# jayHuggie/PathTracer_CUDA_Interactive

Hardware: AMD Instinct MI355X
Metric: Msamples/sec (rays x spp x bounces = intersect() calls per second), scenes/cbox/cbox.xml 640x480 spp=64 (higher is better)
Workload: dtype f32

## Files before the change

pathtracer_cuda_interactive_amd/csrc/pt_kernels.h:

```cpp
#pragma once

#include <hip/hip_runtime.h>

#include <type_traits>

#include "pt_layout.h"
#include "pt_leaf_sweep.h"
#include "pt_math.h"
#include "pt_path_bank.h"
#include "pt_sweep_layout.h"
#include "pt_temporal.h"
#include "pt_trace.h"

namespace ptk {

using namespace ptl;


#ifndef PT_BLOCK
#define PT_BLOCK 256
#endif
constexpr int kBlock = PT_BLOCK;
constexpr uint32_t kMaxChunk = 256;

__device__ __forceinline__ uint32_t lane_rank(unsigned long long mask) {
    return __builtin_amdgcn_mbcnt_hi((uint32_t)(mask >> 32), __builtin_amdgcn_mbcnt_lo((uint32_t)mask, 0u));
}

__device__ __forceinline__ unsigned long long wave_sum(unsigned long long v) {
    for (int off = 32; off > 0; off >>= 1) v += __shfl_down(v, off, 64);
    return v;
}


constexpr int kCounterStride = 32;

struct WorkFeed {
    uint32_t cur, end;
    uint32_t region;
    uint32_t tried;
    bool exhausted;
};

__device__ __forceinline__ uint32_t region_rows(const RenderDev& rp, uint32_t region) {
    const uint32_t first = region * (uint32_t)rp.rows_per_region;
    const uint32_t nrows = (uint32_t)rp.num_rows;
    return first >= nrows ? 0u : min((uint32_t)rp.rows_per_region, nrows - first);
}

__device__ __forceinline__ void feed_init(WorkFeed& f, const RenderDev& rp) {
    f.cur = 0; f.end = 0; f.tried = 0; f.exhausted = false;
    const uint32_t xcc = (uint32_t)__builtin_amdgcn_s_getreg(6164) & 15u;
    f.region = xcc % (uint32_t)rp.num_regions;
}

__device__ __forceinline__ void feed_reserve(WorkFeed& f, const RenderDev& rp, uint32_t* work_counters, int lane) {
    while (f.cur >= f.end && !f.exhausted) {
        const uint32_t total = region_rows(rp, f.region) * (uint32_t)rp.width * (uint32_t)rp.spp_pass;
        const uint32_t chunk = rp.chunk;
        uint32_t base = 0;
        if (lane == 0) base = atomicAdd(&work_counters[f.region * kCounterStride], chunk);
        base = __builtin_amdgcn_readfirstlane(base);
        if (base < total) {
            f.cur = base;
            f.end = min(base + chunk, total);
        } else if (++f.tried >= (uint32_t)rp.num_regions) {
            f.exhausted = true;
        } else {
            f.region = (f.region + 1) % (uint32_t)rp.num_regions;
        }
    }
}

struct PathStart {
    ptd::Ray ray;
    ptm::Pcg rng;
    uint32_t sample_index;
};

struct PathIndex {
    int col, j;
    int32_t img_width;
    uint64_t stream;
    uint32_t sample_index;
};

template <bool LIST = false>
__device__ __forceinline__ PathIndex path_index(const RenderDev& rp, uint32_t region, uint32_t item) {
    const uint32_t npix_r = region_rows(rp, region) * (uint32_t)rp.width;
    uint32_t s_local, rr;
    int i;
    if (rp.row_major) {
        const uint32_t row_s = fastdiv(item, rp.div_width);
        i = (int)(item - row_s * (uint32_t)rp.width);
        rr = fastdiv(row_s, rp.div_spp);
        s_local = row_s - rr * (uint32_t)rp.spp_pass;
    } else {
        s_local = fastdiv(item, (int)region == rp.short_region ? rp.div_npix_last : rp.div_npix_full);
        const uint32_t pix_r = item - s_local * npix_r;
        rr = fastdiv(pix_r, rp.div_width);
        i = (int)(pix_r - rr * (uint32_t)rp.width);
    }
    const uint32_t local_row = region * (uint32_t)rp.rows_per_region + rr;
    uint32_t img_row = local_row;
    int col = i;
    if (LIST) {
        const uint32_t e = rp.list[local_row];
        img_row = fastdiv(e, rp.div_img_width);
        col = (int)(e - img_row * (uint32_t)rp.img_width);
    }
    const int32_t img_width = LIST ? rp.img_width : rp.width;
    const int j = rp.row_begin + (int)img_row * rp.row_step;
    const uint64_t pixel_index = (uint64_t)j * (uint64_t)img_width + (uint64_t)col;
    PathIndex px;
    px.col = col;
    px.j = j;
    px.img_width = img_width;
    px.stream = pixel_index * (uint64_t)rp.stream_stride + (uint64_t)(rp.sample_base + (int)s_local);
    px.sample_index = s_local * rp.npix + local_row * (uint32_t)rp.width + (uint32_t)i;
    return px;
}

template <bool LIST = false>
__device__ __forceinline__ PathStart start_path(const RenderDev& rp, uint32_t region, uint32_t item) {
    const PathIndex px = path_index<LIST>(rp, region, item);
    PathStart ps;
    ps.rng = ptm::pcg_init(px.stream, rp.seed);
    const float ru = ptm::pcg_float(ps.rng);
    const float u = ((float)px.col + ru) / (float)px.img_width;
    const float rv = ptm::pcg_float(ps.rng);
    const float v = ((float)px.j + rv) / (float)rp.height;
    ps.ray = ptd::primary_ray(rp, u, v);
    ps.sample_index = px.sample_index;
    return ps;
}

struct TraceKernelArgs {
    SceneDev scn; RenderDev rp; LdsPlan lp; float4* samples; uint32_t* work_counter; unsigned long long* counters;
};
template <bool WORDS>
__device__ __forceinline__ RenderDev reload_render_args() {
    typedef const __attribute__((address_space(4))) unsigned char* KernargPtr;
    KernargPtr p = (KernargPtr)__builtin_amdgcn_kernarg_segment_ptr();
    asm volatile("" : "+s"(p));
    if (WORDS) {
        struct Words { uint32_t w[sizeof(RenderDev) / 4]; };
        typedef const __attribute__((address_space(4))) uint32_t* WordPtr;
        WordPtr q = (WordPtr)(p + offsetof(TraceKernelArgs, rp));
        Words v;
#pragma unroll
        for (uint32_t i = 0; i < sizeof(RenderDev) / 4; i++) v.w[i] = q[i];
        return __builtin_bit_cast(RenderDev, v);
    }
    RenderDev r;
    __builtin_memcpy(&r, (const void*)(p + offsetof(TraceKernelArgs, rp)), sizeof(RenderDev));
    return r;
}

#ifndef PT_PATH_BANK
#define PT_PATH_BANK 1
#endif
constexpr bool path_bank_on(int res, int spec, bool nee, bool list, int thresh, int inner) {
    return PT_PATH_BANK && (res == 1 || res == 2) && spec == 2 && !nee && !list && thresh == 40 && inner == 162;
}

__device__ __forceinline__ void stage_to_lds(void* dst, const void* src, uint32_t bytes) {
    float4* d = reinterpret_cast<float4*>(dst);
    const float4* s = reinterpret_cast<const float4*>(src);
    for (uint32_t i = threadIdx.x; i < bytes / 16; i += blockDim.x) d[i] = s[i];
}

#ifndef PT_LDS_NODE_STRIDE
#define PT_LDS_NODE_STRIDE 64
#endif
constexpr uint32_t kLdsNodeStride = PT_LDS_NODE_STRIDE;
__device__ __forceinline__ void stage_nodes_to_lds(void* dst, const DNode* src, uint32_t n) {
    const float4* s = reinterpret_cast<const float4*>(src);
    for (uint32_t i = threadIdx.x; i < n * 4; i += blockDim.x)
        *reinterpret_cast<float4*>(reinterpret_cast<unsigned char*>(dst) + (i >> 2) * kLdsNodeStride + (i & 3) * 16) = s[i];
}

template <int RES>
__device__ __forceinline__ ptd::SceneView make_scene_view(const SceneDev& scn, const LdsPlan& lp, unsigned char* smem) {
    ptd::SceneView sv;
    sv.top_nodes = nullptr;
    sv.top_count = 0;
    if (RES == 1 || RES == 2) {
        const uint32_t oct_pitch = oct_table_pitch((uint32_t)scn.num_nodes, kLdsNodeStride);
        if (RES == 2) {
            for (uint32_t o = 0; o < 8; o++)
                stage_nodes_to_lds(smem + lp.nodes_off + o * oct_pitch, scn.nodes_oct + (size_t)o * scn.num_nodes, (uint32_t)scn.num_nodes);
        } else {
            stage_nodes_to_lds(smem + lp.nodes_off, scn.nodes, (uint32_t)scn.num_nodes);
        }
        stage_to_lds(smem + lp.prims_off, scn.prims, (uint32_t)scn.num_prims * sizeof(DPrim));
        stage_to_lds(smem + lp.normals_off, scn.normals, (uint32_t)scn.num_prims * sizeof(DNormals));
        stage_to_lds(smem + lp.mats_off, scn.materials, (uint32_t)scn.num_materials * sizeof(DMaterial));
        stage_to_lds(smem + lp.emis_off, scn.emission, (uint32_t)scn.num_emission * sizeof(DEmission));
        __syncthreads();
        sv.nodes = reinterpret_cast<const DNode*>(smem + lp.nodes_off);
        sv.prims = reinterpret_cast<const DPrim*>(smem + lp.prims_off);
        sv.normals = reinterpret_cast<const DNormals*>(smem + lp.normals_off);
        sv.materials = reinterpret_cast<const DMaterial*>(smem + lp.mats_off);
        sv.emission = reinterpret_cast<const DEmission*>(smem + lp.emis_off);
        sv.node_stride = kLdsNodeStride;
        sv.oct_stride = RES == 2 ? oct_pitch : 0u;
    } else {
        if (RES == 3) {
            stage_to_lds(smem + lp.nodes_off, scn.nodes, lp.top_count * (uint32_t)sizeof(DNode));
            __syncthreads();
            sv.top_nodes = reinterpret_cast<const DNode*>(smem + lp.nodes_off);
            sv.top_count = lp.top_count;
        }
        sv.nodes = scn.nodes; sv.prims = scn.prims; sv.normals = scn.normals;
        sv.materials = scn.materials; sv.emission = scn.emission;
        sv.node_stride = sizeof(DNode);
        sv.oct_stride = 0;
    }
    sv.lights = scn.lights;
    sv.num_emission = scn.num_emission;
    sv.root_ref = scn.root_ref;
    sv.fixed_order = scn.fixed_order;
    sv.ref_nodes = scn.ref_nodes; sv.ref_path = scn.ref_path; sv.ref_anc = scn.ref_anc; sv.ref_levels = scn.ref_levels;
    sv.bg = ptm::mk(scn.bg[0], scn.bg[1], scn.bg[2]);
    return sv;
}

constexpr int kCounterSlots = 64;
constexpr int kSlotStride = 16;
constexpr int kTimelineBase = kCounterSlots * kSlotStride;
constexpr int kNumCounters = kTimelineBase + 8 + 2 * 128;

__device__ __forceinline__ unsigned long long* counter_slot(unsigned long long* counters) {
    return counters + (blockIdx.x % kCounterSlots) * kSlotStride;
}

template <bool STATS>
__device__ __forceinline__ void flush_counters(unsigned long long* counters, int lane, uint32_t n_paths, uint32_t n_segs,
                                               const ptd::TravStats& st) {
    const unsigned long long a = wave_sum(n_paths), b = wave_sum(n_segs);
    const unsigned long long c = STATS ? wave_sum(st.nodes) : 0ull, d = STATS ? wave_sum(st.leaves) : 0ull;
    if (lane == 0) {
        unsigned long long* slot = counter_slot(counters);
        atomicAdd(&slot[0], a);
        atomicAdd(&slot[1], b);
        if (STATS) { atomicAdd(&slot[2], c); atomicAdd(&slot[3], d); }
    }
}

template <bool LDS_SCENE, bool PRUNE, bool STATS, bool LIST = false>
__global__ __launch_bounds__(kBlock) void trace_kernel(SceneDev scn, RenderDev rp, LdsPlan lp,
                                                       float4* __restrict__ samples,
                                                       uint32_t* __restrict__ work_counter,
                                                       unsigned long long* __restrict__ counters) {
    extern __shared__ __attribute__((aligned(16))) unsigned char smem[];
    const ptd::SceneView sv = make_scene_view<(LDS_SCENE ? 1 : 0)>(scn, lp, smem);

    const int lane = threadIdx.x & 63;
    const int wave = threadIdx.x >> 6;
    int32_t* stk = reinterpret_cast<int32_t*>(smem + lp.stack_off) + (size_t)wave * scn.stack_cap * 64 + lane;

    WorkFeed feed;
    feed_init(feed, rp);
    bool alive = false;
    ptd::Ray ray;
    ptm::V3 L = ptm::mk(0, 0, 0), T = ptm::mk(1, 1, 1);
    ptm::Pcg rng;
    rng.state = 0; rng.inc = 1;
    int depth = 0;
    uint32_t my_w = 0;
    uint32_t n_paths = 0, n_segs = 0;
    ptd::TravStats st;
    st.nodes = 0; st.leaves = 0;
    ray.org = ptm::mk(0, 0, 0); ray.dir = ptm::mk(0, 0, 1); ray.tnear = 0; ray.tfar = 0;

    for (;;) {
        const unsigned long long need = __ballot(!alive);
        if (need) {
            feed_reserve(feed, rp, work_counter, lane);
            const uint32_t avail = feed.end - feed.cur;
            if (avail) {
                const uint32_t rank = lane_rank(need);
                const uint32_t n = (uint32_t)__popcll(need);
                if (!alive && rank < avail) {
                    const PathStart ps = start_path<LIST>(rp, feed.region, feed.cur + rank);
                    ray = ps.ray;
                    rng = ps.rng;
                    my_w = ps.sample_index;
                    L = ptm::mk(0, 0, 0);
                    T = ptm::mk(1, 1, 1);
                    depth = 0;
                    alive = true;
                    n_paths++;
                }
                feed.cur += min(n, avail);
            }
        }
        if (!__any(alive)) {
            if (feed.exhausted) break;
            continue;
        }
        if (alive) {
            n_segs++;
            const ptd::Hit h = ptd::intersect<PRUNE, STATS>(sv, ray, stk, st);
            bool cont = false;
            if (h.prim < 0) {
                L = L + T * sv.bg;
            } else {
                const ptd::Surface sf = ptd::make_surface<false>(sv, ray, h);
                cont = ptd::shade_and_bounce<false>(sv, sf, ray, rng, L, T, depth, rp.rr_depth);
                depth++;
                if (depth >= rp.max_depth) cont = false;
            }
            if (!cont) {
                samples[my_w] = make_float4(L.x, L.y, L.z, 0.0f);
                alive = false;
            }
// ... 399 lines not shown
```

pathtracer_cuda_interactive_amd/csrc/pt_trace.h:

```cpp
#pragma once

#include <float.h>

#include "pt_layout.h"
#include "pt_math.h"
#include "pt_reg_stack.h"

namespace ptd {

using namespace ptm;
using namespace ptl;

struct Ray {
    V3 org, dir;
    float tnear, tfar;
};

struct Hit {
    float t, u, v;
    int32_t prim;
};

struct TravStats {
    uint32_t nodes, leaves;
// ... 76 lines not shown
    s.reset(t);
    t.redo = false;
    const uint32_t oct = (t.inv.x < 0.0f ? 1u : 0u) | (t.inv.y < 0.0f ? 2u : 0u) | (t.inv.z < 0.0f ? 4u : 0u);
    t.node_off = oct * sv.oct_stride;
}

__device__ __forceinline__ void slab_distances(const float4 a, const float4 b, const float4 c, const V3& o, const V3& inv,
                                               float& ltn, float& ltf, float& rtn, float& rtf) {
    const bool sx = inv.x < 0.0f, sy = inv.y < 0.0f, sz = inv.z < 0.0f;
    float l0x = (a.x - o.x) * inv.x, l1x = (a.w - o.x) * inv.x;
    float l0y = (a.y - o.y) * inv.y, l1y = (b.x - o.y) * inv.y;
    float l0z = (a.z - o.z) * inv.z, l1z = (b.y - o.z) * inv.z;
    ltn = fmax2(fmax2(sx ? l1x : l0x, sy ? l1y : l0y), sz ? l1z : l0z);
    ltf = fmin2(fmin2(sx ? l0x : l1x, sy ? l0y : l1y), sz ? l0z : l1z);
    float r0x = (b.z - o.x) * inv.x, r1x = (c.y - o.x) * inv.x;
    float r0y = (b.w - o.y) * inv.y, r1y = (c.z - o.y) * inv.y;
    float r0z = (c.x - o.z) * inv.z, r1z = (c.w - o.z) * inv.z;
    rtn = fmax2(fmax2(sx ? r1x : r0x, sy ? r1y : r0y), sz ? r1z : r0z);
    rtf = fmin2(fmin2(sx ? r0x : r1x, sy ? r0y : r1y), sz ? r0z : r1z);
}

template <bool PRUNE, bool OCT, class S>
__device__ __forceinline__ void visit_node(const float4 a, const float4 b, const float4 c, const float4 d, const V3& o, Trav& t, const S& s,
                                           const bool fixed_order) {
    const V3 inv = t.inv;
    float ltn, ltf, rtn, rtf;
    if (OCT) {
        ltn = fmax2(fmax2((a.x - o.x) * inv.x, (a.y - o.y) * inv.y), (a.z - o.z) * inv.z);
        ltf = fmin2(fmin2((a.w - o.x) * inv.x, (b.x - o.y) * inv.y), (b.y - o.z) * inv.z);
        rtn = fmax2(fmax2((b.z - o.x) * inv.x, (b.w - o.y) * inv.y), (c.x - o.z) * inv.z);
        rtf = fmin2(fmin2((c.y - o.x) * inv.x, (c.z - o.y) * inv.y), (c.w - o.z) * inv.z);
    } else {
        slab_distances(a, b, c, o, inv, ltn, ltf, rtn, rtf);
    }
    bool hl = ltf >= fmax2(0.0f, ltn);
    bool hr = rtf >= fmax2(0.0f, rtn);
    if (PRUNE) {
        const float lim = t.best.t + t.best.t * 1e-5f;
        hl = hl && !(ltn > lim);
        hr = hr && !(rtn > lim);
    }
    const int32_t L = __builtin_bit_cast(int32_t, d.x);
    const int32_t R = __builtin_bit_cast(int32_t, d.y);
    const bool left_first = S::kLeftFirst || fixed_order || ltn < rtn;
    const bool both = hl && hr;
    const int32_t next = (hl && (!hr || left_first)) ? L : R;
    s.advance(t, both, hl || hr, next, left_first ? R : L);
}

typedef float f4v __attribute__((ext_vector_type(4)));
typedef __attribute__((address_space(3))) const f4v lds_f4v;

template <class P>
__device__ __forceinline__ void ld_node_lds(const P* p, float4& a, float4& b, float4& c, float4& d) {
    const lds_f4v* nd = (const lds_f4v*)p;
    const f4v va = nd[0], vb = nd[1], vc = nd[2], vd = nd[3];
    a = make_float4(va.x, va.y, va.z, va.w); b = make_float4(vb.x, vb.y, vb.z, vb.w);
    c = make_float4(vc.x, vc.y, vc.z, vc.w); d = make_float4(vd.x, vd.y, vd.z, vd.w);
}

template <bool PRUNE, bool OCT, int TOP = 0, class S>
__device__ __forceinline__ void inner_step(const SceneView& sv, const V3& o, Trav& t, const S& s) {
    float4 a, b, c, d;
    if (TOP == 1 && (uint32_t)t.cur < sv.top_count) {
        ld_node_lds(reinterpret_cast<const unsigned char*>(sv.top_nodes) + (uint32_t)t.cur * (uint32_t)sizeof(DNode), a, b, c, d);
    } else {
        const void* nd = reinterpret_cast<const unsigned char*>(sv.nodes) + (OCT ? t.node_off : 0u) + (uint32_t)t.cur * sv.node_stride;
        a = ld4(nd, 0);
        b = ld4(nd, 1);
        c = ld4(nd, 2);
        d = ld4(nd, 3);
    }
    visit_node<PRUNE, OCT>(a, b, c, d, o, t, s, sv.fixed_order != 0);
}

__device__ __forceinline__ bool ref_visits_first(const SceneView& sv, const V3& o, const V3& inv, const int32_t a, const int32_t b) {
    const unsigned long long pa = sv.ref_path[a], pb = sv.ref_path[b];
    const int level = __builtin_ctzll(pa ^ pb);
    const int32_t node = sv.ref_anc[(size_t)a * (size_t)sv.ref_levels + level];
    const DNode* nd = sv.ref_nodes + node;
    float ltn, ltf, rtn, rtf;
    slab_distances(ld4(nd, 0), ld4(nd, 1), ld4(nd, 2), o, inv, ltn, ltf, rtn, rtf);
    const bool left_first = ltn < rtn;
    const bool b_left = ((pb >> level) & 1ull) == 0ull;
    return b_left == left_first;
}

template <bool TRI_ONLY>
__device__ __forceinline__ void leaf_test(const SceneView& sv, const Ray& ray, Trav& t, const int32_t ref, const bool ties) {
    const int32_t prim = ~ref;
    const DPrim* pr = sv.prims + prim;
    const float4 a = ld4(pr, 0);
    const float4 b = ld4(pr, 1);
    const float4 c = ld4(pr, 2);
    const V3 o = ray.org;
    const int32_t info = __builtin_bit_cast(int32_t, c.y);
    if (TRI_ONLY || info >= 0) {
        const V3 p0 = mk(a.x, a.y, a.z), p1 = mk(a.w, b.x, b.y), p2 = mk(b.z, b.w, c.x);
        const V3 e1 = p1 - p0;
        const V3 e2 = p2 - p0;
        const V3 s1 = cross(ray.dir, e2);
        const float divisor = dot(s1, e1);
        if (divisor != 0.0f) {
            const float inv_divisor = rcp_exact(divisor);
            const V3 s = o - p0;
            const float u = dot(s, s1) * inv_divisor;
            const V3 s2 = cross(s, e1);
            const float v = dot(ray.dir, s2) * inv_divisor;
            const float tt = dot(e2, s2) * inv_divisor;
            if (tt > ray.tnear && tt < ray.tfar && u >= 0.0f && v >= 0.0f && u + v <= 1.0f) {
                bool take = tt < t.best.t;
                if (ties && tt == t.best.t && t.best.prim >= 0) {
                    take = ref_visits_first(sv, o, t.inv, t.best.prim, prim);
                }
                if (take) { t.best.t = tt; t.best.u = u; t.best.v = v; t.best.prim = prim; }
            }
        }
    } else {
        const V3 center = mk(a.x, a.y, a.z);
        const float radius = a.w;
        const V3 vv = o - center;
        const float A = dot(ray.dir, ray.dir);
        const float B = 2.0f * dot(ray.dir, vv);
        const float C = dot(vv, vv) - radius * radius;
        float t0 = 0.0f, t1 = 0.0f;
        bool ok = true;
        if (A == 0.0f) {
            if (B == 0.0f) ok = false;
            else { t0 = -C / B; t1 = t0; }
        } else {
            const float disc = B * B - 4.0f * A * C;
            if (disc < 0.0f) ok = false;
            else {
                const float rd = __builtin_sqrtf(disc);
                if (B >= 0.0f) { t0 = (-B - rd) / (2.0f * A); t1 = 2.0f * C / (-B - rd); }
                else { t0 = 2.0f * C / (-B + rd); t1 = (-B + rd) / (2.0f * A); }
            }
        }
        if (ok) {
            if (t0 > t1) { const float tmp = t0; t0 = t1; t1 = tmp; }
            float tt = t0;
            if (t1 >= ray.tnear && t1 < ray.tfar && tt < ray.tnear) tt = t1;
            if (tt >= ray.tnear && tt < ray.tfar) {
                bool take = tt < t.best.t;
                if (ties && tt == t.best.t && t.best.prim >= 0) take = ref_visits_first(sv, o, t.inv, t.best.prim, prim);
                if (take) { t.best.t = tt; t.best.u = 0.0f; t.best.v = 0.0f; t.best.prim = prim; }
            }
        }
    }
}

__device__ __forceinline__ uint32_t leaf_test_slot(const SceneView& sv, const lds_f4v* slots, const Ray& ray, Trav& t, const uint32_t slot) {
    typedef const __attribute__((address_space(3))) unsigned char* LdsBytes;
    static_assert(sizeof(DPrim) == 48, "slot * 48 as two shift-adds (the compiler's own choice is a 64-bit multiply-add)");
    const lds_f4v* pr = (const lds_f4v*)(((LdsBytes)slots + (slot << 5)) + (slot << 4));
    const f4v a = pr[0], b = pr[1], c = pr[2];
    const float link_bits = c.w;
    const uint32_t link = __builtin_bit_cast(uint32_t, link_bits);
    const int32_t prim = (int32_t)(link & 0xffu);
    const V3 o = ray.org;
    const V3 p0 = mk(a.x, a.y, a.z), e1 = mk(a.w, b.x, b.y), e2 = mk(b.z, b.w, c.x);
    const V3 s1 = cross(ray.dir, e2);
    const float divisor = dot(s1, e1);
    if (divisor != 0.0f) {
        const float inv_divisor = rcp_exact(divisor);
        const V3 s = o - p0;
        const float u = dot(s, s1) * inv_divisor;
        const V3 s2 = cross(s, e1);
        const float v = dot(ray.dir, s2) * inv_divisor;
        const float tt = dot(e2, s2) * inv_divisor;
        if (tt > ray.tnear && u >= 0.0f && v >= 0.0f && u + v <= 1.0f) {
            bool take = tt < t.best.t;
            if (tt == t.best.t && t.best.prim >= 0) {
                float dx = ray.dir.x, dy = ray.dir.y, dz = ray.dir.z;
                asm volatile("" : "+v"(dx), "+v"(dy), "+v"(dz));
                const V3 inv = mk(rcp_exact(dx), rcp_exact(dy), rcp_exact(dz));
                take = ref_visits_first(sv, o, inv, t.best.prim, prim);
            }
            if (take) { t.best.t = tt; t.best.u = u; t.best.v = v; t.best.prim = prim; }
        }
    }
    return link >> 8;
}

template <bool TRI_ONLY, bool ANYHIT = false, class S>
__device__ __forceinline__ void leaf_step(const SceneView& sv, const Ray& ray, Trav& t, const S& s, const bool shadow = false,
                                          const bool ties = false) {
    leaf_test<TRI_ONLY>(sv, ray, t, t.cur, ties);
    if (ANYHIT && shadow && t.best.prim >= 0) s.reset(t);
    s.pop(t);
}

template <bool PRUNE, bool STATS>
__device__ __forceinline__ Hit intersect(const SceneView& sv, const Ray& ray, int32_t* stk, TravStats& st) {
    Trav t;
    const LdsStack<int32_t> s{stk};
    stack_init(stk);
    trav_begin(sv, ray, t, s);
    while (t.cur != kDone) {
        while (t.cur >= 0) {
            if (STATS) st.nodes++;
            inner_step<PRUNE, false>(sv, ray.org, t, s);
        }
        if (t.cur != kDone) {
            if (STATS) st.leaves++;
            leaf_step<false>(sv, ray, t, s);
        }
    }
    return t.best;
}

template <bool PRUNE = false>
__device__ __forceinline__ Hit intersect_any_tree(const SceneView& sv, const SceneView& sv_ref, const Ray& ray, int32_t* stk, bool& rerun) {
    Trav t;
    TravStats st;
    st.nodes = 0; st.leaves = 0;
    const LdsStack<int32_t> s{stk};
    stack_init(stk);
    trav_begin(sv, ray, t, s);
    if (!(__builtin_isfinite(t.inv.x) && __builtin_isfinite(t.inv.y) && __builtin_isfinite(t.inv.z))) {
        t.redo = true;
        t.cur = kDone;
    }
    while (t.cur != kDone) {
        while (t.cur >= 0) inner_step<PRUNE, false>(sv, ray.org, t, s);
        if (t.cur != kDone) leaf_step<false>(sv, ray, t, s, false, true);
    }
    rerun = t.redo;
    return t.redo ? intersect<false, false>(sv_ref, ray, stk, st) : t.best;
}

struct Surface {
    V3 p, n;
    int32_t material, light;
};

template <bool TRI_ONLY>
__device__ __forceinline__ Surface make_surface(const SceneView& sv, const Ray& ray, const Hit& h) {
    Surface s;
    const DPrim* pr = sv.prims + h.prim;
    const float4 a = ld4(pr, 0);
    const float4 b = ld4(pr, 1);
    const float4 c = ld4(pr, 2);
    const int32_t info = __builtin_bit_cast(int32_t, c.y);
    s.material = info & 0x7fffffff;
    s.light = __builtin_bit_cast(int32_t, c.z);
    if (TRI_ONLY || info >= 0) {
        const V3 p0 = mk(a.x, a.y, a.z), p1 = mk(a.w, b.x, b.y), p2 = mk(b.z, b.w, c.x);
        const float w = 1.0f - h.u - h.v;
        s.p = p0 * w + p1 * h.u + p2 * h.v;
        const DNormals* nr = sv.normals + h.prim;
        const float4 na = ld4(nr, 0);
        const float4 nb = ld4(nr, 1);
        const float4 nc = ld4(nr, 2);
        const V3 n0 = mk(na.x, na.y, na.z), n1 = mk(na.w, nb.x, nb.y), n2 = mk(nb.z, nb.w, nc.x);
        s.n = normalize(n0 * w + n1 * h.u + n2 * h.v);
    } else {
        const V3 center = mk(a.x, a.y, a.z);
        s.p = ray.org + ray.dir * h.t;
        s.n = normalize(s.p - center);
    }
    return s;
}

__device__ __forceinline__ V3 to_world_about(V3 n, V3 local) {
    V3 fx, fy;
    if (n.z < float(-1 + 1e-6)) {
        fx = mk(0.0f, -1.0f, 0.0f);
        fy = mk(-1.0f, 0.0f, 0.0f);
    } else {
        const float a = rcp_exact(1.0f + n.z);
        const float b = -n.x * n.y * a;
        fx = mk(1.0f - n.x * n.x * a, b, -n.x);
        fy = mk(b, 1.0f - n.y * n.y * a, -n.y);
    }
    return fx * local.x + fy * local.y + n * local.z;
}

__device__ __forceinline__ V3 reflect_about(V3 wi, V3 n) {
    const float k = 2.0f * dot(wi, n);
    return (-wi) + n * k;
}

__device__ __forceinline__ V3 schlick(V3 F0, float cos_theta) {
    const float p5 = pow5(1.0f - cos_theta);
    return F0 + (mk(1.0f, 1.0f, 1.0f) - F0) * p5;
}

__device__ __forceinline__ V3 sample_cos_hemisphere(float ux, float uy) {
    const float phi = kTwoPi * ux;
    const float tmp = sqrt_exact(clamp01(1.0f - uy));
    float sn, cs;
    sincos_det(phi, sn, cs);
    return mk(cs * tmp, sn * tmp, sqrt_exact(clamp01(uy)));
}

__device__ __forceinline__ V3 sample_cos_n_hemisphere(float ux, float uy, float exponent) {
    const float phi = kTwoPi * ux;
    const float cos_theta = pow_det(uy, 1.0f / (exponent + 1.0f));
    const float sin_theta = __builtin_sqrtf(clamp01(1.0f - cos_theta * cos_theta));
    float sn, cs;
    sincos_det(phi, sn, cs);
    return mk(cs * sin_theta, sn * sin_theta, cos_theta);
}

struct LightSample {
    V3 wl;
    float tfar;
// ... 231 lines not shown
```

pathtracer_cuda_interactive_amd/csrc/pt_trace_sweep_body.h:

```cpp
    extern __shared__ __attribute__((aligned(16))) unsigned char smem[];
    constexpr int THRESH = PT_SWEEP_THRESH;
    typedef const __attribute__((address_space(3))) unsigned char* LdsBytes;
    typedef float f2v __attribute__((ext_vector_type(2)));
    typedef const __attribute__((address_space(3))) f2v* LdsF2;
    const uint32_t n_groups = sweep.groups;
    const uint32_t box_pitch = sweep_box_pitch(n_groups);
    const ptd::SceneView sv = make_sweep_view(scn, lp, sweep, smem);
    const ptd::lds_f4v* slots = (const ptd::lds_f4v*)(smem + lp.nodes_off + sweep_slots_off(n_groups));

    const int lane = threadIdx.x & 63;
    const int wave = threadIdx.x >> 6;

    WorkFeed feed;
    feed_init(feed, rp);
    PathBank bank;
    bank_init(bank);
    float bank_dx = 0.0f, bank_dy = 0.0f, bank_dz = 0.0f;
    uint32_t bank_lo = 0, bank_hi = 0;
    bool alive = false;
    ptd::Ray ray;
    ray.org = ptm::mk(0, 0, 0); ray.dir = ptm::mk(0, 0, 1); ray.tnear = 0; ray.tfar = 0;
    ptd::Trav tv;
    tv.inv = ptm::mk(1, 1, 1);
    tv.best.t = 0; tv.best.u = 0; tv.best.v = 0; tv.best.prim = -1;
    tv.cur = 0; tv.stack_state = 0; tv.node_off = 0; tv.redo = false;
    uint32_t hits = 0;
    uint32_t pend = 0;
    ptm::V3 L = ptm::mk(0, 0, 0), T = ptm::mk(1, 1, 1);
    ptm::Pcg rng;
    rng.state = 0; rng.inc = 1;
    int depth = 0;
    uint32_t my_w = 0;
    uint32_t n_paths = 0, n_segs = 0;
    ptd::TravStats st;
    st.nodes = 0; st.leaves = 0;
    ptd::SceneView sv_ref = sv;
    sv_ref.nodes = scn.ref_nodes; sv_ref.root_ref = scn.ref_root_ref; sv_ref.node_stride = sizeof(DNode);
    sv_ref.oct_stride = 0; sv_ref.top_nodes = nullptr; sv_ref.top_count = 0; sv_ref.fixed_order = 0;
    int32_t* redo_stk = scn.redo_stack + ((size_t)(blockIdx.x * (kBlock / 64) + wave) * (size_t)scn.redo_cap) * 64 + lane;

    for (;;) {
        const bool idle = (hits | pend) == 0u;
        const unsigned long long idle_mask = __ballot(idle);
        const bool work_left = bank_work_left(bank, feed.exhausted, feed.cur, feed.end);
        const int n_pend = __popcll(__ballot(idle && (alive || work_left)));
        if (n_pend >= THRESH || idle_mask == ~0ull) {
            if (n_pend == 0) break;
            if (idle && alive && tv.redo) {
                ptd::TravStats st_redo;
                st_redo.nodes = 0; st_redo.leaves = 0;
                ray.tfar = depth == 0 ? __builtin_inff() : FLT_MAX;
                tv.best = ptd::intersect<false, false>(sv_ref, ray, redo_stk, st_redo);
                tv.redo = false;
            }
            if (idle && alive) {
                bool cont = false;
                if (tv.best.prim < 0) {
                    L = L + T * sv.bg;
                } else {
                    const ptd::Surface sf = ptd::make_surface<true>(sv, ray, tv.best);
                    cont = ptd::shade_and_bounce<true, false>(sv, sf, ray, rng, L, T, depth, rp.rr_depth, nullptr);
                    depth++;
                    if (depth >= rp.max_depth) cont = false;
                }
                if (!cont) {
                    samples[my_w] = make_float4(L.x, L.y, L.z, 0.0f);
                    alive = false;
                }
            }
            unsigned long long want = __ballot(idle && !alive);
#pragma nounroll
            for (int round = 0; round < 2 && want; round++) {
                if (bank.left == 0) {
                    feed_reserve(feed, rp, work_counter, lane);
                    if (feed.cur >= feed.end) break;
                    bank_fill(bank, feed.cur, feed.end);
                    const RenderDev rg = reload_render_args<false>();
                    const PathStart ps = start_path<false>(rg, feed.region, bank_item(feed.cur, (uint32_t)lane));
                    bank_dx = ps.ray.dir.x; bank_dy = ps.ray.dir.y; bank_dz = ps.ray.dir.z;
                    bank_lo = (uint32_t)ps.rng.state; bank_hi = (uint32_t)(ps.rng.state >> 32);
                }
                uint32_t first;
                const uint32_t k = bank_take(bank, (uint32_t)__popcll(want), first);
                const uint32_t rank = lane_rank(want);
                const bool take = idle && !alive && rank < k;
                const int src = take ? (int)(first + rank) : lane;
                const float dx = __shfl(bank_dx, src, 64), dy = __shfl(bank_dy, src, 64), dz = __shfl(bank_dz, src, 64);
                const uint32_t lo = __shfl(bank_lo, src, 64), hi = __shfl(bank_hi, src, 64);
                if (take) {
                    const PathIndex px = path_index<false>(rp, feed.region, bank_item(feed.cur, first + rank));
                    ray.org = ptm::mk(rp.cam_origin[0], rp.cam_origin[1], rp.cam_origin[2]);
                    ray.dir = ptm::mk(dx, dy, dz);
                    ray.tnear = 0.0f;
                    rng.state = (uint64_t)hi << 32 | lo;
                    rng.inc = (px.stream << 1u) | 1u;
                    my_w = px.sample_index;
                    L = ptm::mk(0, 0, 0);
                    T = ptm::mk(1, 1, 1);
                    depth = 0;
                    alive = true;
                }
                n_paths += k;
                want = __ballot(idle && !alive);
            }
            n_segs += (uint32_t)__popcll(__ballot(idle && alive));
            if (idle && alive) {
                const ptm::V3 inv = ptm::mk(ptm::rcp_exact(ray.dir.x), ptm::rcp_exact(ray.dir.y), ptm::rcp_exact(ray.dir.z));
                tv.best.t = FLT_MAX; tv.best.u = 0.0f; tv.best.v = 0.0f; tv.best.prim = -1;
                tv.redo = !(__builtin_isfinite(inv.x) && __builtin_isfinite(inv.y) && __builtin_isfinite(inv.z));
                if (!tv.redo) {
                    const uint32_t oct = (inv.x < 0.0f ? 1u : 0u) | (inv.y < 0.0f ? 2u : 0u) | (inv.z < 0.0f ? 4u : 0u);
                    LdsF2 bx = (LdsF2)((LdsBytes)smem + lp.nodes_off + oct * box_pitch);
                    const ptm::V3 o = ray.org;
                    auto box_hit = [&](const f2v p0, const f2v p1, const f2v p2) -> uint32_t {
                        const float tn = ptm::fmax2(ptm::fmax2((p0.x - o.x) * inv.x, (p0.y - o.y) * inv.y), (p1.x - o.z) * inv.z);
                        const float tf = ptm::fmin2(ptm::fmin2((p1.y - o.x) * inv.x, (p2.x - o.y) * inv.y), (p2.y - o.z) * inv.z);
                        return tf >= ptm::fmax2(0.0f, tn) ? 1u : 0u;
                    };
                    uint32_t h = 0;
#pragma clang loop vectorize(disable) interleave(disable) unroll(disable)
                    for (uint32_t k = n_groups >> 1; k != 0; k--) {
                        const f2v a0 = bx[0], a1 = bx[1], a2 = bx[2], b0 = bx[3], b1 = bx[4], b2 = bx[5];
                        bx += 6;
                        h = 2u * h + box_hit(a0, a1, a2);
                        h = 2u * h + box_hit(b0, b1, b2);
                    }
                    if (n_groups & 1u) h = 2u * h + box_hit(bx[0], bx[1], bx[2]);
                    hits = sweep_hits_align(h, n_groups);
                }
            }
        }
#pragma unroll
        for (int k = 0; k < N_LEAF; k++) {
            if ((hits | pend) != 0u) {
                uint32_t slot = pend;
                if (pend == 0u) {
                    slot = sweep_first_group(hits);
                    hits = sweep_clear_group(hits, slot);
                }
                pend = ptd::leaf_test_slot(sv, slots, ray, tv, slot);
            }
        }
    }
    flush_counters<false>(counters, lane, lane == 0 ? n_paths : 0u, lane == 0 ? n_segs : 0u, st);
```

pathtracer_cuda_interactive_amd/csrc/pt_trace_v2_body.h:

```cpp
    extern __shared__ __attribute__((aligned(16))) unsigned char smem[];
    const unsigned long long tl_entry = STATS ? wall_clock64() : 0ull;
    const ptd::SceneView sv = make_scene_view<RES>(scn, lp, smem);
    const unsigned long long tl_staged = STATS ? wall_clock64() : 0ull;
    unsigned long long tl_dry = 0;

    constexpr bool TRI_ONLY = SPEC >= 1, DIFFUSE_ONLY = SPEC >= 2;
    using STK = typename std::conditional<RES == 1 || RES == 2, int16_t, int32_t>::type;
    using STACK = typename std::conditional<REG, ptd::RegStack, ptd::LdsStack<STK>>::type;
    static_assert(!REG || ((RES == 1 || RES == 2) && THRESH == 40 && INNER == 162), "RegStack: see reg_stack_on");
    constexpr int32_t DONE = STACK::kDone;
    constexpr bool POSTPONE = INNER >= 1000;
    constexpr int BURST = INNER >= 1000 ? INNER - 1000 : INNER;
    int32_t pend = DONE;
    const int lane = threadIdx.x & 63;
    const int wave = threadIdx.x >> 6;
    STACK stack;
    if constexpr (!REG) stack.col = reinterpret_cast<STK*>(smem + lp.stack_off) + (size_t)wave * scn.stack_cap * 64 + lane;

    WorkFeed feed;
    feed_init(feed, rp);
    constexpr bool BANK = path_bank_on(RES, SPEC, NEE, LIST, THRESH, INNER);
    PathBank bank;
    bank_init(bank);
    float bank_dx = 0.0f, bank_dy = 0.0f, bank_dz = 0.0f;
    uint32_t bank_lo = 0, bank_hi = 0;
    bool alive = false;
    ptd::Ray ray;
    ray.org = ptm::mk(0, 0, 0); ray.dir = ptm::mk(0, 0, 1); ray.tnear = 0; ray.tfar = 0;
    ptd::Trav tv;
    tv.inv = ptm::mk(1, 1, 1);
    tv.best.t = 0; tv.best.u = 0; tv.best.v = 0; tv.best.prim = -1;
    tv.cur = DONE; tv.node_off = 0; tv.redo = false;
    stack.reset(tv);
    if constexpr (!REG) ptd::stack_init(stack.col);
    ptm::V3 L = ptm::mk(0, 0, 0), T = ptm::mk(1, 1, 1);
    ptm::Pcg rng;
    rng.state = 0; rng.inc = 1;
    int depth = 0;
    uint32_t my_w = 0;
    uint32_t n_paths = 0, n_segs = 0;
    ptd::TravStats st;
    st.nodes = 0; st.leaves = 0;
    const bool fbk = scn.fallback != 0;
    ptd::SceneView sv_ref = sv;
    sv_ref.nodes = scn.ref_nodes; sv_ref.root_ref = scn.ref_root_ref; sv_ref.node_stride = sizeof(DNode);
    sv_ref.oct_stride = 0; sv_ref.top_nodes = nullptr; sv_ref.top_count = 0; sv_ref.fixed_order = 0;
    int32_t* redo_stk = scn.redo_stack + ((size_t)(blockIdx.x * (kBlock / 64) + wave) * (size_t)scn.redo_cap) * 64 + lane;
    uint32_t n_redo = 0;
    ptd::NeeState nee;
    nee.count_emission = true; nee.want_shadow = false;
    nee.ls.wl = ptm::mk(0, 0, 1); nee.ls.tfar = 0; nee.ls.contrib = ptm::mk(0, 0, 0);
    bool in_shadow = false, cont_after = false;
    ptm::V3 next_dir = ptm::mk(0, 0, 1);

    unsigned long long dg_iter = 0, dg_sched = 0, dg_sched_lanes = 0, dg_in = 0, dg_in_lanes = 0, dg_lf = 0, dg_lf_lanes = 0, dg_wait = 0;

    for (;;) {
        const bool idle = tv.cur == DONE && (!POSTPONE || pend == DONE);
        const unsigned long long idle_mask = __ballot(idle);
        if (STATS) dg_iter++;
        const bool work_left = BANK ? bank_work_left(bank, feed.exhausted, feed.cur, feed.end) : !(feed.exhausted && feed.cur >= feed.end);
        if (STATS && !work_left && tl_dry == 0) tl_dry = wall_clock64();
        const int n_pend = __popcll(__ballot(idle && (alive || work_left)));
        int thresh = THRESH;
        if ((RES == 0 || RES == 3) && !work_left) thresh = min(THRESH, max(1, (__popcll(__ballot(alive)) + 3) / 4));
        if (n_pend >= thresh || idle_mask == ~0ull) {
            if (n_pend == 0) break;
            if (STATS) { dg_sched++; dg_sched_lanes += (unsigned)n_pend; }
            if (fbk && idle && alive && tv.redo) {
                ptd::TravStats st_redo;
                st_redo.nodes = 0; st_redo.leaves = 0;
                tv.best = ptd::intersect<false, false>(sv_ref, ray, redo_stk, st_redo);
                tv.redo = false;
                if (STATS) n_redo++;
            }
            if (idle && alive) {
                bool cont = false;
                if (NEE && in_shadow) {
                    if (tv.best.prim < 0) L = L + nee.ls.contrib;
                    in_shadow = false;
                    cont = cont_after;
                    if (cont) { ray.dir = next_dir; ray.tnear = 1e-4f; ray.tfar = FLT_MAX; }
                } else if (tv.best.prim < 0) {
                    L = L + T * sv.bg;
                } else {
                    const ptd::Surface sf = ptd::make_surface<TRI_ONLY>(sv, ray, tv.best);
                    cont = ptd::shade_and_bounce<DIFFUSE_ONLY, NEE>(sv, sf, ray, rng, L, T, depth, rp.rr_depth, NEE ? &nee : nullptr);
                    depth++;
                    if (depth >= rp.max_depth) cont = false;
                    if (NEE && nee.want_shadow) {
                        in_shadow = true;
                        cont_after = cont;
                        next_dir = ray.dir;
                        ray.dir = nee.ls.wl; ray.tnear = 1e-4f; ray.tfar = nee.ls.tfar;
                        cont = true;
                    }
                }
                if (!cont) {
                    samples[my_w] = make_float4(L.x, L.y, L.z, 0.0f);
                    alive = false;
                }
            }
            const unsigned long long need = __ballot(idle && !alive);
            if (BANK) {
                unsigned long long want = need;
#pragma nounroll
                for (int round = 0; round < 2 && want; round++) {
                    if (bank.left == 0) {
                        feed_reserve(feed, rp, work_counter, lane);
                        if (feed.cur >= feed.end) break;
                        bank_fill(bank, feed.cur, feed.end);
                        const RenderDev rg = reload_render_args<STATS>();
                        const PathStart ps = start_path<LIST>(rg, feed.region, bank_item(feed.cur, (uint32_t)lane));
                        bank_dx = ps.ray.dir.x; bank_dy = ps.ray.dir.y; bank_dz = ps.ray.dir.z;
                        bank_lo = (uint32_t)ps.rng.state; bank_hi = (uint32_t)(ps.rng.state >> 32);
                    }
                    uint32_t first;
                    const uint32_t k = bank_take(bank, (uint32_t)__popcll(want), first);
                    const uint32_t rank = lane_rank(want);
                    const bool take = idle && !alive && rank < k;
                    const int src = take ? (int)(first + rank) : lane;
                    const float dx = __shfl(bank_dx, src, 64), dy = __shfl(bank_dy, src, 64), dz = __shfl(bank_dz, src, 64);
                    const uint32_t lo = __shfl(bank_lo, src, 64), hi = __shfl(bank_hi, src, 64);
                    if (take) {
                        const PathIndex px = path_index<LIST>(rp, feed.region, bank_item(feed.cur, first + rank));
                        ray.org = ptm::mk(rp.cam_origin[0], rp.cam_origin[1], rp.cam_origin[2]);
                        ray.dir = ptm::mk(dx, dy, dz);
                        ray.tnear = 0.0f;
                        ray.tfar = __builtin_inff();
                        rng.state = (uint64_t)hi << 32 | lo;
                        rng.inc = (px.stream << 1u) | 1u;
                        my_w = px.sample_index;
                        L = ptm::mk(0, 0, 0);
                        T = ptm::mk(1, 1, 1);
                        depth = 0;
                        alive = true;
                        n_paths++;
                    }
                    want = __ballot(idle && !alive);
                }
            } else if (need) {
                feed_reserve(feed, rp, work_counter, lane);
                const uint32_t avail = feed.end - feed.cur;
                if (avail) {
                    const uint32_t rank = lane_rank(need);
                    const uint32_t n = (uint32_t)__popcll(need);
                    if (idle && !alive && rank < avail) {
                        const PathStart ps = start_path<LIST>(rp, feed.region, feed.cur + rank);
                        ray = ps.ray;
                        rng = ps.rng;
                        my_w = ps.sample_index;
                        L = ptm::mk(0, 0, 0);
                        T = ptm::mk(1, 1, 1);
                        depth = 0;
                        alive = true;
                        n_paths++;
                        if (NEE) { nee.count_emission = true; in_shadow = false; }
                    }
                    feed.cur += min(n, avail);
                }
            }
            if (idle && alive) {
                ptd::trav_begin(sv, ray, tv, stack);
                if (!(NEE && in_shadow)) n_segs++;
                if (fbk && !(__builtin_isfinite(tv.inv.x) && __builtin_isfinite(tv.inv.y) && __builtin_isfinite(tv.inv.z))) {
                    tv.redo = true;
                    tv.cur = DONE;
                }
            }
        }
        if (POSTPONE) {
            constexpr int REPS = BURST >= 100 ? BURST / 100 : 1;
            constexpr int N_IN = BURST >= 100 ? (BURST / 10) % 10 : BURST;
            constexpr int N_LF = BURST >= 100 ? BURST % 10 : 1;
#pragma unroll
            for (int r = 0; r < REPS; r++) {
#pragma unroll
                for (int k = 0; k < N_IN; k++) {
                    if (STATS) {
                        const int n_in = __popcll(__ballot(tv.cur >= 0));
                        if (n_in) { dg_in++; dg_in_lanes += (unsigned)n_in; dg_wait += (unsigned)__popcll(__ballot(tv.cur == DONE && pend == DONE)); }
                    }
                    if (tv.cur >= 0) {
                        if (STATS && !BANK) st.nodes++;
                        ptd::inner_step<PRUNE, RES == 2, (RES == 3 ? 1 : 0)>(sv, ray.org, tv, stack);
                        if (tv.cur < 0 && tv.cur != DONE && pend == DONE) {
                            pend = tv.cur;
                            stack.pop(tv);
                        }
                    }
                }
#pragma unroll
                for (int k = 0; k < N_LF; k++) {
                    if (STATS) {
                        const int n_lf = __popcll(__ballot(pend != DONE));
                        if (n_lf) { dg_lf++; dg_lf_lanes += (unsigned)n_lf; dg_wait += (unsigned)__popcll(__ballot(tv.cur == DONE && pend == DONE)); }
                    }
                    if (pend != DONE) {
                        if (STATS && !BANK) st.leaves++;
                        ptd::leaf_test<TRI_ONLY>(sv, ray, tv, pend, fbk);
                        pend = DONE;
                        if (NEE && in_shadow && tv.best.prim >= 0) { tv.cur = DONE; stack.reset(tv); }
                        if (tv.cur < 0 && tv.cur != DONE) {
                            pend = tv.cur;
                            stack.pop(tv);
                        }
                    }
                }
            }
        } else if (INNER < 0) {
#pragma unroll
            for (int k = 0; k < -INNER; k++) {
                const bool at_inner = tv.cur >= 0;
                const bool at_leaf = tv.cur < 0 && tv.cur != DONE;
                const int n_in = __popcll(__ballot(at_inner));
                const int n_lf = __popcll(__ballot(at_leaf));
                if (STATS && (n_in | n_lf)) {
                    dg_wait += (unsigned)(64 - n_in - n_lf);
                    if (n_in >= n_lf) { dg_in++; dg_in_lanes += (unsigned)n_in; } else { dg_lf++; dg_lf_lanes += (unsigned)n_lf; }
                }
                if (n_in >= n_lf) {
                    if (at_inner) {
                        if (STATS && !BANK) st.nodes++;
                        ptd::inner_step<PRUNE, RES == 2, (RES == 3 ? 1 : 0)>(sv, ray.org, tv, stack);
                    }
                } else if (at_leaf) {
                    if (STATS && !BANK) st.leaves++;
                    ptd::leaf_step<TRI_ONLY, NEE>(sv, ray, tv, stack, NEE && in_shadow, fbk);
                }
            }
        } else {
            constexpr int REPS = INNER >= 100 ? INNER / 100 : 1;
            constexpr int N_IN = INNER >= 100 ? (INNER / 10) % 10 : (INNER > 0 ? INNER : 1);
            constexpr int N_LF = INNER >= 100 ? INNER % 10 : 1;
#pragma unroll
            for (int r = 0; r < REPS; r++) {
#pragma unroll
                for (int k = 0; k < N_IN; k++) {
                    if (STATS) {
                        const int n_in = __popcll(__ballot(tv.cur >= 0));
                        if (n_in) { dg_in++; dg_in_lanes += (unsigned)n_in; dg_wait += (unsigned)__popcll(__ballot(tv.cur == DONE)); }
                    }
                    if (tv.cur >= 0) {
                        if (STATS && !BANK) st.nodes++;
                        ptd::inner_step<PRUNE, RES == 2, (RES == 3 ? 1 : 0)>(sv, ray.org, tv, stack);
                    }
                }
#pragma unroll
                for (int k = 0; k < N_LF; k++) {
                    if (STATS) {
                        const int n_lf = __popcll(__ballot(tv.cur < 0 && tv.cur != DONE));
                        if (n_lf) { dg_lf++; dg_lf_lanes += (unsigned)n_lf; dg_wait += (unsigned)__popcll(__ballot(tv.cur == DONE)); }
                    }
                    if (tv.cur < 0 && tv.cur != DONE) {
                        if (STATS && !BANK) st.leaves++;
                        ptd::leaf_step<TRI_ONLY, NEE>(sv, ray, tv, stack, NEE && in_shadow, fbk);
                    }
                }
            }
        }
    }
    if (BANK && STATS) {
        st.nodes = lane == 0 ? (uint32_t)dg_in_lanes : 0u;
        st.leaves = lane == 0 ? (uint32_t)dg_lf_lanes : 0u;
    }
    flush_counters<STATS>(counters, lane, n_paths, n_segs, st);
    const unsigned long long redo_sum = STATS ? wave_sum(n_redo) : 0ull;
    if (STATS && lane == 0) {
        const unsigned long long tl_exit = wall_clock64();
        unsigned long long* slot = counter_slot(counters);
        atomicAdd(&slot[4], dg_iter); atomicAdd(&slot[5], dg_sched); atomicAdd(&slot[6], dg_sched_lanes);
        atomicAdd(&slot[7], dg_in); atomicAdd(&slot[8], dg_in_lanes); atomicAdd(&slot[9], dg_lf);
        atomicAdd(&slot[10], dg_lf_lanes); atomicAdd(&slot[11], dg_wait);
        atomicAdd(&slot[12], redo_sum);
        unsigned long long* tl = counters + kTimelineBase;
        if (tl_dry == 0) tl_dry = tl_exit;
        atomicMax(&tl[0], ~tl_entry); atomicMax(&tl[1], tl_staged); atomicMax(&tl[2], ~tl_dry);
        atomicMax(&tl[3], tl_dry); atomicMax(&tl[4], tl_exit); atomicAdd(&tl[5], tl_exit - tl_dry);
        atomicAdd(&tl[6], tl_dry - tl_staged); atomicAdd(&tl[7], 1ull);
        atomicAdd(&tl[8 + min(127ull, (tl_dry - tl_entry) / 10000ull)], 1ull);
        atomicAdd(&tl[136 + min(127ull, (tl_exit - tl_entry) / 10000ull)], 1ull);
    }
```

Baseline: 42170.

## Bank path index and rng increment, asm carry-chain box hits, simpler slot addressing

Path-bank refills now precompute each lane's sample index and PCG increment and hand them out with shuffles, so a path start no longer recomputes path_index with its fastdiv work. The sweep body's box-hit bitmask is built with inline-asm compare plus add-with-carry instead of select-and-shift. LDS primitive slot addressing becomes a 32-bit multiply, with an assume on the slot bound. The change adds three shuffles per refill and live registers, and uses hand-written asm with s_nop hazard padding.

```diff
diff --git a/pathtracer_cuda_interactive_amd/csrc/pt_kernels.h b/pathtracer_cuda_interactive_amd/csrc/pt_kernels.h
--- a/pathtracer_cuda_interactive_amd/csrc/pt_kernels.h
+++ b/pathtracer_cuda_interactive_amd/csrc/pt_kernels.h
@@ -8,6 +8,7 @@
 #include "pt_leaf_sweep.h"
 #include "pt_math.h"
 #include "pt_path_bank.h"
+#include "pt_path_index.h"
 #include "pt_sweep_layout.h"
 #include "pt_temporal.h"
 #include "pt_trace.h"
@@ -41,12 +42,6 @@
     uint32_t tried;
     bool exhausted;
 };
-
-__device__ __forceinline__ uint32_t region_rows(const RenderDev& rp, uint32_t region) {
-    const uint32_t first = region * (uint32_t)rp.rows_per_region;
-    const uint32_t nrows = (uint32_t)rp.num_rows;
-    return first >= nrows ? 0u : min((uint32_t)rp.rows_per_region, nrows - first);
-}
 
 __device__ __forceinline__ void feed_init(WorkFeed& f, const RenderDev& rp) {
     f.cur = 0; f.end = 0; f.tried = 0; f.exhausted = false;
@@ -77,49 +72,6 @@
     ptm::Pcg rng;
     uint32_t sample_index;
 };
-
-struct PathIndex {
-    int col, j;
-    int32_t img_width;
-    uint64_t stream;
-    uint32_t sample_index;
-};
-
-template <bool LIST = false>
-__device__ __forceinline__ PathIndex path_index(const RenderDev& rp, uint32_t region, uint32_t item) {
-    const uint32_t npix_r = region_rows(rp, region) * (uint32_t)rp.width;
-    uint32_t s_local, rr;
-    int i;
-    if (rp.row_major) {
-        const uint32_t row_s = fastdiv(item, rp.div_width);
-        i = (int)(item - row_s * (uint32_t)rp.width);
-        rr = fastdiv(row_s, rp.div_spp);
-        s_local = row_s - rr * (uint32_t)rp.spp_pass;
-    } else {
-        s_local = fastdiv(item, (int)region == rp.short_region ? rp.div_npix_last : rp.div_npix_full);
-        const uint32_t pix_r = item - s_local * npix_r;
-        rr = fastdiv(pix_r, rp.div_width);
-        i = (int)(pix_r - rr * (uint32_t)rp.width);
-    }
-    const uint32_t local_row = region * (uint32_t)rp.rows_per_region + rr;
-    uint32_t img_row = local_row;
-    int col = i;
-    if (LIST) {
-        const uint32_t e = rp.list[local_row];
-        img_row = fastdiv(e, rp.div_img_width);
-        col = (int)(e - img_row * (uint32_t)rp.img_width);
-    }
-    const int32_t img_width = LIST ? rp.img_width : rp.width;
-    const int j = rp.row_begin + (int)img_row * rp.row_step;
-    const uint64_t pixel_index = (uint64_t)j * (uint64_t)img_width + (uint64_t)col;
-    PathIndex px;
-    px.col = col;
-    px.j = j;
-    px.img_width = img_width;
-    px.stream = pixel_index * (uint64_t)rp.stream_stride + (uint64_t)(rp.sample_base + (int)s_local);
-    px.sample_index = s_local * rp.npix + local_row * (uint32_t)rp.width + (uint32_t)i;
-    return px;
-}
 
 template <bool LIST = false>
 __device__ __forceinline__ PathStart start_path(const RenderDev& rp, uint32_t region, uint32_t item) {
@@ -163,6 +115,8 @@
 constexpr bool path_bank_on(int res, int spec, bool nee, bool list, int thresh, int inner) {
     return PT_PATH_BANK && (res == 1 || res == 2) && spec == 2 && !nee && !list && thresh == 40 && inner == 162;
 }
+
+constexpr bool bank_index_on(bool reg, bool stats, int minw) { return minw <= 5 && (reg || !stats); }
 
 __device__ __forceinline__ void stage_to_lds(void* dst, const void* src, uint32_t bytes) {
     float4* d = reinterpret_cast<float4*>(dst);
diff --git a/pathtracer_cuda_interactive_amd/csrc/pt_path_index.h b/pathtracer_cuda_interactive_amd/csrc/pt_path_index.h
--- /dev/null
+++ b/pathtracer_cuda_interactive_amd/csrc/pt_path_index.h
@@ -0,0 +1,76 @@
+#pragma once
+#include <stdint.h>
+
+#include "pt_layout.h"
+
+#if defined(__HIPCC__)
+#define PT_PIDX_HD __host__ __device__ __forceinline__
+#else
+#define PT_PIDX_HD inline
+#endif
+
+namespace ptl {
+
+PT_PIDX_HD uint32_t region_rows(const RenderDev& rp, uint32_t region) {
+    const uint32_t first = region * (uint32_t)rp.rows_per_region;
+    const uint32_t nrows = (uint32_t)rp.num_rows;
+    const uint32_t rest = nrows - first;
+    return first >= nrows ? 0u : ((uint32_t)rp.rows_per_region < rest ? (uint32_t)rp.rows_per_region : rest);
+}
+
+struct PathIndex {
+    int col, j;
+    int32_t img_width;
+    uint64_t stream;
+    uint32_t sample_index;
+};
+
+template <bool LIST = false>
+PT_PIDX_HD PathIndex path_index(const RenderDev& rp, uint32_t region, uint32_t item) {
+    const uint32_t npix_r = region_rows(rp, region) * (uint32_t)rp.width;
+    uint32_t s_local, rr;
+    int i;
+    if (rp.row_major) {
+        const uint32_t row_s = fastdiv(item, rp.div_width);
+        i = (int)(item - row_s * (uint32_t)rp.width);
+        rr = fastdiv(row_s, rp.div_spp);
+        s_local = row_s - rr * (uint32_t)rp.spp_pass;
+    } else {
+        s_local = fastdiv(item, (int)region == rp.short_region ? rp.div_npix_last : rp.div_npix_full);
+        const uint32_t pix_r = item - s_local * npix_r;
+        rr = fastdiv(pix_r, rp.div_width);
+        i = (int)(pix_r - rr * (uint32_t)rp.width);
+    }
+    const uint32_t local_row = region * (uint32_t)rp.rows_per_region + rr;
+    uint32_t img_row = local_row;
+    int col = i;
+    if (LIST) {
+        const uint32_t e = rp.list[local_row];
+        img_row = fastdiv(e, rp.div_img_width);
+        col = (int)(e - img_row * (uint32_t)rp.img_width);
+    }
+    const int32_t img_width = LIST ? rp.img_width : rp.width;
+    const int j = rp.row_begin + (int)img_row * rp.row_step;
+    const uint64_t pixel_index = (uint64_t)j * (uint64_t)img_width + (uint64_t)col;
+    PathIndex px;
+    px.col = col;
+    px.j = j;
+    px.img_width = img_width;
+    px.stream = pixel_index * (uint64_t)rp.stream_stride + (uint64_t)(rp.sample_base + (int)s_local);
+    px.sample_index = s_local * rp.npix + local_row * (uint32_t)rp.width + (uint32_t)i;
+    return px;
+}
+
+PT_PIDX_HD uint64_t stream_inc(uint64_t stream) { return (stream << 1u) | 1u; }
+
+struct BankIndex {
+    uint32_t sample_index, inc_lo, inc_hi;
+};
+PT_PIDX_HD BankIndex bank_index_pack(uint32_t sample_index, uint64_t inc) {
+    BankIndex b;
+    b.sample_index = sample_index; b.inc_lo = (uint32_t)inc; b.inc_hi = (uint32_t)(inc >> 32);
+    return b;
+}
+PT_PIDX_HD uint64_t bank_index_inc(uint32_t inc_lo, uint32_t inc_hi) { return (uint64_t)inc_hi << 32 | inc_lo; }
+
+}
diff --git a/pathtracer_cuda_interactive_amd/csrc/pt_trace.h b/pathtracer_cuda_interactive_amd/csrc/pt_trace.h
--- a/pathtracer_cuda_interactive_amd/csrc/pt_trace.h
+++ b/pathtracer_cuda_interactive_amd/csrc/pt_trace.h
@@ -252,8 +252,9 @@
 
 __device__ __forceinline__ uint32_t leaf_test_slot(const SceneView& sv, const lds_f4v* slots, const Ray& ray, Trav& t, const uint32_t slot) {
     typedef const __attribute__((address_space(3))) unsigned char* LdsBytes;
-    static_assert(sizeof(DPrim) == 48, "slot * 48 as two shift-adds (the compiler's own choice is a 64-bit multiply-add)");
-    const lds_f4v* pr = (const lds_f4v*)(((LdsBytes)slots + (slot << 5)) + (slot << 4));
+    static_assert(sizeof(DPrim) == 48 && ptl::kSweepMaxPrims * sizeof(DPrim) < (1u << 24), "slot * 48 in 24 bits");
+    __builtin_assume(slot < (uint32_t)ptl::kSweepMaxPrims);
+    const lds_f4v* pr = (const lds_f4v*)((LdsBytes)slots + slot * (uint32_t)sizeof(DPrim));
     const f4v a = pr[0], b = pr[1], c = pr[2];
     const float link_bits = c.w;
     const uint32_t link = __builtin_bit_cast(uint32_t, link_bits);
diff --git a/pathtracer_cuda_interactive_amd/csrc/pt_trace_sweep_body.h b/pathtracer_cuda_interactive_amd/csrc/pt_trace_sweep_body.h
--- a/pathtracer_cuda_interactive_amd/csrc/pt_trace_sweep_body.h
+++ b/pathtracer_cuda_interactive_amd/csrc/pt_trace_sweep_body.h
@@ -17,6 +17,7 @@
     bank_init(bank);
     float bank_dx = 0.0f, bank_dy = 0.0f, bank_dz = 0.0f;
     uint32_t bank_lo = 0, bank_hi = 0;
+    uint32_t bank_w = 0, bank_inc_lo = 0, bank_inc_hi = 0;
     bool alive = false;
     ptd::Ray ray;
     ray.org = ptm::mk(0, 0, 0); ray.dir = ptm::mk(0, 0, 1); ray.tnear = 0; ray.tfar = 0;
@@ -79,6 +80,8 @@
                     const PathStart ps = start_path<false>(rg, feed.region, bank_item(feed.cur, (uint32_t)lane));
                     bank_dx = ps.ray.dir.x; bank_dy = ps.ray.dir.y; bank_dz = ps.ray.dir.z;
                     bank_lo = (uint32_t)ps.rng.state; bank_hi = (uint32_t)(ps.rng.state >> 32);
+                    const BankIndex bi = bank_index_pack(ps.sample_index, ps.rng.inc);
+                    bank_w = bi.sample_index; bank_inc_lo = bi.inc_lo; bank_inc_hi = bi.inc_hi;
                 }
                 uint32_t first;
                 const uint32_t k = bank_take(bank, (uint32_t)__popcll(want), first);
@@ -87,14 +90,14 @@
                 const int src = take ? (int)(first + rank) : lane;
                 const float dx = __shfl(bank_dx, src, 64), dy = __shfl(bank_dy, src, 64), dz = __shfl(bank_dz, src, 64);
                 const uint32_t lo = __shfl(bank_lo, src, 64), hi = __shfl(bank_hi, src, 64);
+                const uint32_t w = __shfl(bank_w, src, 64), inc_lo = __shfl(bank_inc_lo, src, 64), inc_hi = __shfl(bank_inc_hi, src, 64);
                 if (take) {
-                    const PathIndex px = path_index<false>(rp, feed.region, bank_item(feed.cur, first + rank));
                     ray.org = ptm::mk(rp.cam_origin[0], rp.cam_origin[1], rp.cam_origin[2]);
                     ray.dir = ptm::mk(dx, dy, dz);
                     ray.tnear = 0.0f;
                     rng.state = (uint64_t)hi << 32 | lo;
-                    rng.inc = (px.stream << 1u) | 1u;
-                    my_w = px.sample_index;
+                    rng.inc = bank_index_inc(inc_lo, inc_hi);
+                    my_w = w;
                     L = ptm::mk(0, 0, 0);
                     T = ptm::mk(1, 1, 1);
                     depth = 0;
@@ -112,20 +115,32 @@
                     const uint32_t oct = (inv.x < 0.0f ? 1u : 0u) | (inv.y < 0.0f ? 2u : 0u) | (inv.z < 0.0f ? 4u : 0u);
                     LdsF2 bx = (LdsF2)((LdsBytes)smem + lp.nodes_off + oct * box_pitch);
                     const ptm::V3 o = ray.org;
-                    auto box_hit = [&](const f2v p0, const f2v p1, const f2v p2) -> uint32_t {
+                    auto box_sides = [&](const f2v p0, const f2v p1, const f2v p2, float& tf, float& tn0) {
                         const float tn = ptm::fmax2(ptm::fmax2((p0.x - o.x) * inv.x, (p0.y - o.y) * inv.y), (p1.x - o.z) * inv.z);
-                        const float tf = ptm::fmin2(ptm::fmin2((p1.y - o.x) * inv.x, (p2.x - o.y) * inv.y), (p2.y - o.z) * inv.z);
-                        return tf >= ptm::fmax2(0.0f, tn) ? 1u : 0u;
+                        tf = ptm::fmin2(ptm::fmin2((p1.y - o.x) * inv.x, (p2.x - o.y) * inv.y), (p2.y - o.z) * inv.z);
+                        tn0 = ptm::fmax2(0.0f, tn);
                     };
                     uint32_t h = 0;
 #pragma clang loop vectorize(disable) interleave(disable) unroll(disable)
                     for (uint32_t k = n_groups >> 1; k != 0; k--) {
                         const f2v a0 = bx[0], a1 = bx[1], a2 = bx[2], b0 = bx[3], b1 = bx[4], b2 = bx[5];
                         bx += 6;
-                        h = 2u * h + box_hit(a0, a1, a2);
-                        h = 2u * h + box_hit(b0, b1, b2);
+                        float tfa, tna, tfb, tnb;
+                        box_sides(a0, a1, a2, tfa, tna);
+                        box_sides(b0, b1, b2, tfb, tnb);
+                        unsigned long long mb;
+                        asm("v_cmp_ge_f32_e32 vcc, %2, %3\n\t"
+                            "v_cmp_ge_f32_e64 %1, %4, %5\n\t"
+                            "s_nop 0\n\t"
+                            "v_addc_co_u32_e32 %0, vcc, %0, %0, vcc\n\t"
+                            "v_addc_co_u32_e64 %0, vcc, %0, %0, %1"
+                            : "+v"(h), "=&s"(mb) : "v"(tfa), "v"(tna), "v"(tfb), "v"(tnb) : "vcc");
                     }
-                    if (n_groups & 1u) h = 2u * h + box_hit(bx[0], bx[1], bx[2]);
+                    if (n_groups & 1u) {
+                        float tf, tn0;
+                        box_sides(bx[0], bx[1], bx[2], tf, tn0);
+                        asm("v_cmp_ge_f32_e32 vcc, %1, %2\n\ts_nop 1\n\tv_addc_co_u32_e32 %0, vcc, %0, %0, vcc" : "+v"(h) : "v"(tf), "v"(tn0) : "vcc");
+                    }
                     hits = sweep_hits_align(h, n_groups);
                 }
             }
diff --git a/pathtracer_cuda_interactive_amd/csrc/pt_trace_v2_body.h b/pathtracer_cuda_interactive_amd/csrc/pt_trace_v2_body.h
--- a/pathtracer_cuda_interactive_amd/csrc/pt_trace_v2_body.h
+++ b/pathtracer_cuda_interactive_amd/csrc/pt_trace_v2_body.h
@@ -24,6 +24,8 @@
     bank_init(bank);
     float bank_dx = 0.0f, bank_dy = 0.0f, bank_dz = 0.0f;
     uint32_t bank_lo = 0, bank_hi = 0;
+    constexpr bool BANK_INDEX = BANK && bank_index_on(REG, STATS, MINW);
+    uint32_t bank_w = 0, bank_inc_lo = 0, bank_inc_hi = 0;
     bool alive = false;
     ptd::Ray ray;
     ray.org = ptm::mk(0, 0, 0); ray.dir = ptm::mk(0, 0, 1); ray.tnear = 0; ray.tfar = 0;
@@ -114,6 +116,10 @@
                         const PathStart ps = start_path<LIST>(rg, feed.region, bank_item(feed.cur, (uint32_t)lane));
                         bank_dx = ps.ray.dir.x; bank_dy = ps.ray.dir.y; bank_dz = ps.ray.dir.z;
                         bank_lo = (uint32_t)ps.rng.state; bank_hi = (uint32_t)(ps.rng.state >> 32);
+                        if constexpr (BANK_INDEX) {
+                            const BankIndex bi = bank_index_pack(ps.sample_index, ps.rng.inc);
+                            bank_w = bi.sample_index; bank_inc_lo = bi.inc_lo; bank_inc_hi = bi.inc_hi;
+                        }
                     }
                     uint32_t first;
                     const uint32_t k = bank_take(bank, (uint32_t)__popcll(want), first);
@@ -122,15 +128,24 @@
                     const int src = take ? (int)(first + rank) : lane;
                     const float dx = __shfl(bank_dx, src, 64), dy = __shfl(bank_dy, src, 64), dz = __shfl(bank_dz, src, 64);
                     const uint32_t lo = __shfl(bank_lo, src, 64), hi = __shfl(bank_hi, src, 64);
+                    uint32_t w = 0, inc_lo = 0, inc_hi = 0;
+                    if constexpr (BANK_INDEX) {
+                        w = __shfl(bank_w, src, 64); inc_lo = __shfl(bank_inc_lo, src, 64); inc_hi = __shfl(bank_inc_hi, src, 64);
+                    }
                     if (take) {
-                        const PathIndex px = path_index<LIST>(rp, feed.region, bank_item(feed.cur, first + rank));
                         ray.org = ptm::mk(rp.cam_origin[0], rp.cam_origin[1], rp.cam_origin[2]);
                         ray.dir = ptm::mk(dx, dy, dz);
                         ray.tnear = 0.0f;
                         ray.tfar = __builtin_inff();
                         rng.state = (uint64_t)hi << 32 | lo;
-                        rng.inc = (px.stream << 1u) | 1u;
-                        my_w = px.sample_index;
+                        if constexpr (BANK_INDEX) {
+                            rng.inc = bank_index_inc(inc_lo, inc_hi);
+                            my_w = w;
+                        } else {
+                            const PathIndex px = path_index<LIST>(rp, feed.region, bank_item(feed.cur, first + rank));
+                            rng.inc = stream_inc(px.stream);
+                            my_w = px.sample_index;
+                        }
                         L = ptm::mk(0, 0, 0);
                         T = ptm::mk(1, 1, 1);
                         depth = 0;
```

Result: faster. 44240 (median of 6 runs) (+4.9%).
